# radhofan/Fairify

Measured on AMD Instinct MI355X. Metric: % partitions verified + partitions/sec on AC suite at 1/2/4/8 MI355X, higher is better.
Workload: dtype fp32

## Files before the change

### fairify_amd/csrc/bindings.cpp

```cpp
#include <hip/hip_runtime.h>
#include <pybind11/pybind11.h>
#include <pybind11/stl.h>

#include <cmath>
#include <cstring>
#include <cstdint>
#include <stdexcept>
#include <vector>

#include "runtime_host.h"

namespace py = pybind11;

extern "C" int fa_bounds_launch(const NetDesc& net, BoundArgs args, hipStream_t stream);
extern "C" int fa_crown_phase_launch(const NetDesc& net, CrownPhaseArgs a, hipStream_t stream);
extern "C" size_t fa_crown_phase_bytes(const NetDesc& net);
extern "C" int fa_point_try_launch(const NetDesc& net, BoundArgs a, hipStream_t stream);
extern "C" int fa_forward_launch(const NetDesc& net, FwdArgs a, hipStream_t stream);
extern "C" int fa_sim_launch(const NetDesc& net, SimArgs a, hipStream_t stream);
extern "C" int fa_sim_shaped(const NetDesc& net);
extern "C" int fa_rate_launch(const NetDesc& net, RateArgs a, hipStream_t stream);
extern "C" int fa_ascent_launch(const NetDesc& net, AscentArgs a, hipStream_t stream);
extern "C" int fa_certify_launch(CertArgs a, hipStream_t stream);
extern "C" int fa_falsify_launch(const NetDesc& net, FalsifyArgs a, hipStream_t stream);
// ... 84 lines not shown
  }
  int n_params;
  int total_floats;
};

const NetDesc& fa_net_desc(py::handle h) { return h.cast<const Net&>().d; }
void register_bab(py::module& m);
void register_relu(py::module& m);
void register_beta(py::module& m);
extern "C" int fa_crown_launch(const NetDesc& net, BoundArgs a, hipStream_t stream);
extern "C" int fa_refine_launch(const NetDesc& net, BoundArgs a, hipStream_t stream);
extern "C" int fa_backward_launch(const NetDesc& net, BoundArgs a, hipStream_t stream);
extern "C" int fa_refine_crown_launch(const NetDesc& net, BoundArgs a, hipStream_t stream);
void register_csv(py::module& m);

using fa_rt::ckl;

PYBIND11_MODULE(_C, m) {
  m.doc() = "fairify_amd CDNA4 (gfx950) kernels";
  py::class_<Net>(m, "Net")
      .def(py::init<const std::vector<int>&, double>())
      .def_readonly("n_params", &Net::n_params)
      .def_readonly("total_floats", &Net::total_floats)
      .def_property_readonly("wperm_off", [](const Net& n) { return n.d.wperm_off; })
      .def_property_readonly("pack_g", [](const Net& n) { return n.d.pack_g; })
      .def_property_readonly("pack_off", [](const Net& n) { return n.d.pack_off; })
      .def_property_readonly("n_hidden", [](const Net& n) { return n.d.n_hidden; })
      .def_property_readonly("n_neurons", [](const Net& n) { return n.d.n_neurons; });

  m.def("bounds", [](const Net& net, uintptr_t flat, uintptr_t lo, uintptr_t hi, uintptr_t dead_in, int R,
                     int symbolic, uintptr_t out_lb, uintptr_t out_ub, uintptr_t Lc, uintptr_t L0, uintptr_t Le,
                     uintptr_t Uc, uintptr_t U0, uintptr_t Ue, uintptr_t layer_lb, uintptr_t layer_ub,
                     uintptr_t dead_out, int G, uintptr_t stream, unsigned long long fold, uintptr_t phase_in,
                     uintptr_t infeas) {
    NetDesc d = net.d;
    BoundArgs a{};
    a.flat = P<const float>(flat);
    a.lo = P<const float>(lo);
    a.hi = P<const float>(hi);
    a.dead_in = P<const uint8_t>(dead_in);
    a.R = R;
    a.symbolic = symbolic;
    a.G = G;
    a.out_lb = P<float>(out_lb);
    a.out_ub = P<float>(out_ub);
    a.Lc = P<float>(Lc); a.L0 = P<float>(L0); a.Le = P<float>(Le);
    a.Uc = P<float>(Uc); a.U0 = P<float>(U0); a.Ue = P<float>(Ue);
    a.layer_lb = P<float>(layer_lb);
    a.layer_ub = P<float>(layer_ub);
    a.dead_out = P<uint8_t>(dead_out);
    a.fold = fold;
    a.phase_in = P<const int8_t>(phase_in);
    a.infeas = P<uint8_t>(infeas);
    ckl(fa_bounds_launch(d, a, (hipStream_t)stream), "bounds");
  }, py::arg("net"), py::arg("flat"), py::arg("lo"), py::arg("hi"), py::arg("dead_in"), py::arg("R"),
     py::arg("symbolic"), py::arg("out_lb"), py::arg("out_ub"), py::arg("Lc"), py::arg("L0"), py::arg("Le"),
     py::arg("Uc"), py::arg("U0"), py::arg("Ue"), py::arg("layer_lb"), py::arg("layer_ub"), py::arg("dead_out"),
     py::arg("G"), py::arg("stream"), py::arg("fold") = 0ull, py::arg("phase_in") = 0, py::arg("infeas") = 0);

  m.def("crown_phase", [](const Net& net, uintptr_t flat, uintptr_t lo, uintptr_t hi, int R, uintptr_t phase,
                          uintptr_t layer_lb, uintptr_t layer_ub, uintptr_t infeas, uintptr_t out_lb, uintptr_t out_ub,
                          uintptr_t Lc, uintptr_t L0, uintptr_t Le, uintptr_t Uc, uintptr_t U0, uintptr_t Ue,
                          uintptr_t split, uintptr_t score, uintptr_t low, uintptr_t stream) {
    CrownPhaseArgs a{};
    a.flat = P<const float>(flat);
    a.lo = P<const float>(lo);
    a.hi = P<const float>(hi);
    a.R = R;
    a.phase = P<const int8_t>(phase);
    a.layer_lb = P<const float>(layer_lb);
    a.layer_ub = P<const float>(layer_ub);
    a.infeas = P<const uint8_t>(infeas);
    a.out_lb = P<float>(out_lb);
    a.out_ub = P<float>(out_ub);
    a.Lc = P<float>(Lc); a.L0 = P<float>(L0); a.Le = P<float>(Le);
    a.Uc = P<float>(Uc); a.U0 = P<float>(U0); a.Ue = P<float>(Ue);
    a.split = P<int>(split);
    a.score = P<float>(score);
    a.low = P<float>(low);
    const int rc = fa_crown_phase_launch(net.d, a, (hipStream_t)stream);
    if (rc != 0) throw std::runtime_error("crown_phase launch failed, code " + std::to_string(rc));
  });

  m.def("relu_fits", [](const Net& net) { return fa_crown_phase_bytes(net.d) > 0; });

  m.def("crown", [](const Net& net, uintptr_t flat, uintptr_t lo, uintptr_t hi, uintptr_t dead_in, int R,
                    uintptr_t out_lb, uintptr_t out_ub, uintptr_t Lc, uintptr_t L0, uintptr_t Le, uintptr_t Uc,
                    uintptr_t U0, uintptr_t Ue, uintptr_t layer_lb, uintptr_t layer_ub, uintptr_t stream) {
    BoundArgs a{};
    a.flat = P<const float>(flat);
    a.lo = P<const float>(lo);
// ... 482 lines not shown
```

### fairify_amd/csrc/symbolic.hip

```cpp
#include <hip/hip_runtime.h>

#include <stdlib.h>

#include <algorithm>
#include <map>
#include <mutex>
#include <tuple>
#include <utility>
#include <vector>

#include "args.h"

#define FA_SYM_MAXC 48

struct SymCfg {
  int nc;
  int cdim[FA_SYM_MAXC];
  unsigned long long fold;
  int w_lds[FA_MAX_LAYERS];
  int b_lds[FA_MAX_LAYERS];
  int lds_floats;
  int stage_off;
  int stage_floats;
};
// ... 19 lines not shown
        if (a->pa_idx[k] == d) x = a->values[v * a->npa + k];
    return x;
  }
};

__device__ __forceinline__ int fa_trot(int rho) { return rho >> 3; }

template <int NT, int PG = 1>
struct SymSlab {
  static constexpr int TS = 16 * NT + 4;
  static constexpr int TILE1 = 2 * 16 * TS;
  static constexpr int TILE = 2 * TILE1;
  static constexpr int BOX = 3 * FA_SYM_MAXC;
  static constexpr int BOXTAB = PG > 1 ? 2 * PG * 32 : 0;
  static constexpr int FLOATS = (TILE + 2 * PG * BOX + BOXTAB + 3) & ~3;
};

template <bool PAIR, int TM>
struct SymForm {
  static constexpr bool CR = !PAIR && TM >= 2;
};

__device__ __forceinline__ void fa_pq_to_ul(const f32x4& P, const f32x4& Q, int fc, float gg, f32x4& U,
                                            f32x4& L) {
  const float sl = (fc == 1 || fc == 3) ? 2.f * gg : 0.f;
#pragma unroll
  for (int i = 0; i < 4; ++i) {
    const float q = Q[i], e = sl * fabsf(q);
    U[i] = (P[i] + q) + e;
    L[i] = (P[i] - q) - e;
  }
}

template <int NT, bool PAIR, int PG = 1, bool CR = false, class S = SymShapeAny>
__device__ __forceinline__ bool fa_sym_epilogue(const NetDesc& net, const BoundArgs& a, const SymCfg& cfg,
                                                const float* smem, float* T, const float* bxv_in, const int* cdim_s,
                                                int l, int r_in, int node_in, int r2, int node2, bool v2, int lane,
                                                int jt0, const f32x4 (&U)[2][NT],
                                                const f32x4 (&Lq)[2][NT], float (&nu)[2][NT][4],
                                                float (&nlo)[2][NT][4]) {
  constexpr int TS = SymSlab<NT>::TS;
  constexpr bool CS = S::L > 0;
  const int col = lane & 15, grp = lane >> 4;
  const int n_out = CS ? S::dim(l + 1) : net.dims[l + 1];
  const float* sb = smem + cfg.b_lds[l];
  const bool last = CS ? l == S::L - 1 : l == net.n_layers - 1;
  const float gg = net.g_gemm[l];
  const float gc = net.g_conc;
  const float gi = net.g_one;
  const float unit = net.unit;
  const float gnext = last ? 0.f : (CR ? net.g_fwd[l + 1] : net.g_gemm[l + 1]);
  const int noff = net.neuron_off[l];
  const int nc = cfg.nc;
  const int n0 = CS ? S::dim(0) : net.dims[0];
  const int tsub = lane >> 5;
  const bool second = PAIR && tsub;
  constexpr int PS = 16 / PG;
  const int gbox = PG > 1 ? col / PS : 0;
  const int bidx = tsub * PG + gbox;
  const int r = PG > 1 ? r_in + bidx : (second ? r2 : r_in);
  const int node = PG > 1 ? (a.V > 0 ? r / a.V : r) : (second ? node2 : node_in);
  const float* bxv = bxv_in + (PG > 1 ? bidx : (second ? 1 : 0)) * SymSlab<NT, PG>::BOX;
  const int jt = PAIR ? jt0 : jt0 + tsub;
  const int n_out_t = n_out;
  const bool nl_act = PG > 1 ? r < a.R : (16 * jt < n_out_t && (!second || v2));
  const int ob = (lane >> 4) & 1;
  float* Trow = T + tsub * SymSlab<NT>::TILE1 + (ob * 16 + col) * TS + fa_trot(ob * 16 + col);
#pragma unroll
    for (int u = 0; u < 2; ++u)
#pragma unroll
      for (int ct = 0; ct < NT; ++ct)
#pragma unroll
        for (int i = 0; i < 4; ++i) {
          const int ru = 4 * grp + i, rl = 16 + 4 * grp + i;
          T[u * SymSlab<NT>::TILE1 + ru * TS + fa_trot(ru) + ct * 16 + col] = U[u][ct][i];
          T[u * SymSlab<NT>::TILE1 + rl * TS + fa_trot(rl) + ct * 16 + col] = Lq[u][ct][i];
        }
    __builtin_amdgcn_wave_barrier();
    const int j = PG > 1 ? col - gbox * PS : 16 * jt + col;
    const bool jv = j < n_out;
    float v[16 * NT];
#pragma unroll
    for (int c = 0; c < 16 * NT; ++c) v[c] = Trow[c];
    const float braw = sb[PG > 1 ? col : min(j, n_out - 1)];
    const float b = jv ? braw : 0.f;
    float s1 = 0.f, s2 = 0.f, mg = 0.f;
#pragma unroll
    for (int c = 4; c < 16 * NT; ++c) {
      const float av = fabsf(v[c]);
      s1 = fmaf(v[c], bxv[c], s1);
      s2 = fmaf(av, bxv[FA_SYM_MAXC + c], s2);
      mg = fmaf(av, bxv[2 * FA_SYM_MAXC + c], mg);
    }
    float mn = s1 - s2, mx = s1 + s2;
    const float cr = v[0];
    float er = v[1], ivr = v[2], ier = v[3];
    const float sgn = ob ? -1.f : 1.f;
    er *= sgn;
    ier *= sgn;
    const float c0 = cr + b;
    const float mgc = mg;
    mn += c0; mx += c0; mg += fabsf(c0);
    const float iv = ivr + b;
    const float eI = ier * (1.f + 2.f * gg) + gg * fabsf(b);
    const float e = er * (1.f + 2.f * gg) + gg * fabsf(b);
    float bound;
    if (ob == 0) bound = fminf(iv + gi * fabsf(iv) + eI, mx + gc * mg + e);
    else bound = fmaxf(iv - gi * fabsf(iv) - eI, mn - gc * mg - e);
    const float other = __shfl_xor(bound, 16, 64);
    const float ub = ob == 0 ? bound : other;
    const float lb = ob == 0 ? other : bound;
    if (nl_act && jv && a.layer_lb) {
      if (ob == 0) a.layer_ub[(size_t)r * net.n_neurons + noff + j] = ub;
      else a.layer_lb[(size_t)r * net.n_neurons + noff + j] = lb;
    }
    if (last) {
      if (nl_act && j == 0) {
        float* Cf = ob == 0 ? a.Uc : a.Lc;
        if (ob == 0) {
          a.out_ub[r] = ub; a.U0[r] = c0; a.Ue[r] = e;
        } else {
          a.out_lb[r] = lb; a.L0[r] = c0; a.Le[r] = e;
        }
        for (int d = 0; d < n0; ++d)
          if ((cfg.fold >> d) & 1ull) Cf[(size_t)r * n0 + d] = 0.f;
        for (int c = 0; c < nc; ++c) Cf[(size_t)r * n0 + cdim_s[c]] = Trow[4 + c];
      }
      return false;
    }
    bool forced = false, fact = false;
    if (nl_act && jv) {
      if (a.dead_in) forced = a.dead_in[(size_t)r * net.n_hidden + noff + j] != 0;
      else if (a.dead_part) forced = a.dead_part[(size_t)a.node_part[node] * net.n_hidden + noff + j] != 0;
      if (a.phase_in) {
        const int8_t ph = a.phase_in[(size_t)r * net.n_hidden + noff + j];
        forced = forced || ph < 0;
        fact = ph > 0;
        if (ob == 0 && a.infeas && ((ph < 0 && lb > 0.f) || (ph > 0 && ub < 0.f))) a.infeas[r] = 1;
      }
    }
    const bool isdead = ub <= 0.f;
    const bool isact = lb >= 0.f;
    if (nl_act && ob == 0 && jv && a.dead_out) a.dead_out[(size_t)r * net.n_hidden + noff + j] = isdead ? 1 : 0;
    const bool zero = isdead || forced || !jv;
    const float aa = mn - gc * mg + e;
    const float bb = mx + gc * mg + e;
    const bool chord = !zero && !isact && !fact && aa < 0.f;
    const float sc = (bb / (bb - aa)) * (1.f + 4.f * unit);
    const float shift = e - aa;
    const float cc = c0 * sc + sc * shift;
    const float sU = zero ? 0.f : (chord ? sc : 1.f);
    const float cU = zero ? 0.f : (chord ? cc : c0);
    const float mU = zero ? 0.f : (chord ? sc * mgc * (1.f + 8.f * unit) + fabsf(cc) : mg);
    const float eU = zero ? 0.f : (chord ? 4.f * unit * sc * (mg + fabsf(shift)) : e);
    const float aL = mn - gc * mg - e;
    const float bL = mx + gc * mg - e;
    const bool lam1 = !zero && (isact || ((bL > 0.f) && (bL > -aL)));
    const bool up = ob == 0;
    const float ivn = zero ? 0.f : fmaxf(up ? ub : lb, 0.f);
    const float s = up ? sU : (lam1 ? 1.f : 0.f);
    const float cnew = up ? cU : (lam1 ? c0 : 0.f);
    const float en = up ? eU : (lam1 ? e : 0.f);
    const float mgn = up ? mU : (lam1 ? mg : 0.f);
    const float mg_b = CR ? mgn + __shfl_xor(mgn, 16, 64) : mgn;
    const float iv_b = CR ? fmaxf(ivn, __shfl_xor(ivn, 16, 64)) : ivn;
    v[0] = cnew;
    v[1] = sgn * (en + gnext * mg_b);
    v[2] = ivn;
    v[3] = sgn * (gnext * iv_b);
#pragma unroll
    for (int c = 4; c < 16 * NT; ++c) v[c] *= s;
    if (nl_act) {
#pragma unroll
      for (int c = 0; c < 16 * NT; ++c) Trow[c] = v[c];
    }
    __builtin_amdgcn_wave_barrier();
#pragma unroll
    for (int u = 0; u < 2; ++u)
#pragma unroll
      for (int ct = 0; ct < NT; ++ct)
#pragma unroll
        for (int i = 0; i < 4; ++i) {
          const int ru = 4 * grp + i, rl = 16 + 4 * grp + i;
          const float xu = T[u * SymSlab<NT>::TILE1 + ru * TS + fa_trot(ru) + ct * 16 + col];
          const float xl = T[u * SymSlab<NT>::TILE1 + rl * TS + fa_trot(rl) + ct * 16 + col];
          nu[u][ct][i] = CR ? 0.5f * (xu + xl) : xu;
          nlo[u][ct][i] = CR ? 0.5f * (xu - xl) : xl;
        }
    __builtin_amdgcn_wave_barrier();
    return true;
}

template <int NT, int TM, bool PAIR, int PG = 1, class S = SymShapeAny>
__device__ __forceinline__ void fa_sym_layer(const NetDesc& net, const BoundArgs& a, const SymCfg& cfg,
                                             const float* smem, float* T, const float* bxv, const int* cdim_s,
                                             int l, int r, int node, int r2, int node2, bool v2, int lane,
                                             const float (&B)[NT][PAIR ? 2 : TM][2][4],
                                             float (&A)[NT][PAIR ? 2 : TM][2][4]) {
  constexpr int TMS = PAIR ? 2 : TM;
  constexpr bool CR = SymForm<PAIR, TM>::CR;
  constexpr int TS = SymSlab<NT>::TS;
  constexpr bool CS = S::L > 0;
  const int col = lane & 15, grp = lane >> 4;
  const int n_in = CS ? S::dim(l) : net.dims[l], n_out = CS ? S::dim(l + 1) : net.dims[l + 1];
  const int tin = (n_in + 15) >> 4, tout = (n_out + 15) >> 4;
  const float* sw = smem + cfg.w_lds[l];
  const float* sb = smem + cfg.b_lds[l];
  const bool last = CS ? l == S::L - 1 : l == net.n_layers - 1;
  const float gg = net.g_gemm[l];
  const float gc = net.g_conc;
  const float gi = net.g_one;
  const float unit = net.unit;
  const float gnext = last ? 0.f : net.g_gemm[l + 1];
  const int noff = net.neuron_off[l];
  const int nc = cfg.nc;
  const int n0 = CS ? S::dim(0) : net.dims[0];
  const bool nl_act = lane < 32;
  const int ob = (lane >> 4) & 1;
#ifndef FA_SYM_TIMING_NO_EPILOGUE
  if (PG > 1 && l == 0) {
    const float* boxtab = bxv + 2 * PG * SymSlab<NT, PG>::BOX;
    const float g0 = net.g_gemm[0];
    const int n0v = n0;
    f32x4 U[2][NT], Lq[2][NT];
#pragma unroll
    for (int u = 0; u < 2; ++u) {
// ... 73 lines not shown
          for (int ct = 0; ct < NT; ++ct) {
            const int bt = PAIR ? bi : t;
            if (CR) {
              su[bi][ct] = fmaf(wv[i], B[ct][bt][0][i], su[bi][ct]);
              sl[bi][ct] = fmaf(fabsf(wv[i]), B[ct][bt][1][i], sl[bi][ct]);
            } else {
              su[bi][ct] = fmaf(wp, B[ct][bt][0][i], fmaf(wn, B[ct][bt][1][i], su[bi][ct]));
              sl[bi][ct] = fmaf(wp, B[ct][bt][1][i], fmaf(wn, B[ct][bt][0][i], sl[bi][ct]));
            }
          }
      }
    }
    f32x4 U[2][NT], Lq[2][NT];
#pragma unroll
    for (int ct = 0; ct < NT; ++ct) U[1][ct] = Lq[1][ct] = f32x4{0.f, 0.f, 0.f, 0.f};
#pragma unroll
    for (int bi = 0; bi < NB; ++bi)
#pragma unroll
      for (int ct = 0; ct < NT; ++ct) {
        float xu = su[bi][ct], xl = sl[bi][ct];
        xu += __shfl_xor(xu, 16, 64);
        xl += __shfl_xor(xl, 16, 64);
        xu += __shfl_xor(xu, 32, 64);
        xl += __shfl_xor(xl, 32, 64);
        U[bi][ct] = f32x4{grp == 0 ? xu : 0.f, 0.f, 0.f, 0.f};
        Lq[bi][ct] = f32x4{grp == 0 ? xl : 0.f, 0.f, 0.f, 0.f};
        if (CR) fa_pq_to_ul(f32x4(U[bi][ct]), f32x4(Lq[bi][ct]), ct * 16 + col, gg, U[bi][ct], Lq[bi][ct]);
      }
    float nu[2][NT][4], nlo[2][NT][4];
    fa_sym_epilogue<NT, PAIR, PG, CR, S>(net, a, cfg, smem, T, bxv, cdim_s, l, r, node, r2, node2, v2, lane, 0, U, Lq,
                                  nu, nlo);
    return;
  }
#endif
#pragma unroll
  for (int jt0 = 0; jt0 < TM; jt0 += 2) {
    if (jt0 >= tout) break;
    f32x4 U[2][NT], Lq[2][NT];
#pragma unroll
    for (int u = 0; u < 2; ++u) {
      const int jt = jt0 + u;
#pragma unroll
      for (int ct = 0; ct < NT; ++ct) {
        U[u][ct] = f32x4{0.f, 0.f, 0.f, 0.f};
        Lq[u][ct] = f32x4{0.f, 0.f, 0.f, 0.f};
      }
      if (PAIR ? (jt0 > 0) : (jt >= tout || jt >= TM)) continue;
      const float4* wq = reinterpret_cast<const float4*>(sw) + (size_t)(PAIR ? 0 : jt) * tin * 64 + lane;
#pragma unroll
      for (int t = 0; t < TM; ++t) {
        if (t >= tin) break;
        const float4 w4 = wq[t * 64];
        const float wv[4] = {w4.x, w4.y, w4.z, w4.w};
#pragma unroll
        for (int i = 0; i < 4; ++i) {
          const float wp = fmaxf(wv[i], 0.f), wn = fminf(wv[i], 0.f);
#pragma unroll
          for (int ct = 0; ct < NT; ++ct) {
            const int bt = PAIR ? u : t;
            const float bu = B[ct][bt][0][i], bl = B[ct][bt][1][i];
            if (CR) {
              U[u][ct] = fa_mfma4(wv[i], bu, U[u][ct]);
              Lq[u][ct] = fa_mfma4(fabsf(wv[i]), bl, Lq[u][ct]);
            } else {
              U[u][ct] = fa_mfma4(wp, bu, U[u][ct]);
              Lq[u][ct] = fa_mfma4(wp, bl, Lq[u][ct]);
// ... 22 lines not shown
        }
    if (l == net.n_layers - 1) {
      if (lane == 0) a.out_lb[r] = nu[0][0][0] + nlo[0][0][1];
      continue;
    }
#else
    if (!fa_sym_epilogue<NT, PAIR, PG, CR, S>(net, a, cfg, smem, T, bxv, cdim_s, l, r, node, r2, node2, v2, lane, jt0, U,
                                       Lq, nu, nlo))
      continue;
#endif
#pragma unroll
    for (int u = 0; u < 2; ++u) {
      if (jt0 + u >= TMS) break;
#pragma unroll
      for (int ct = 0; ct < NT; ++ct)
#pragma unroll
        for (int i = 0; i < 4; ++i) {
          A[ct][jt0 + u][0][i] = nu[u][ct][i];
          A[ct][jt0 + u][1][i] = nlo[u][ct][i];
        }
    }
  }
}

#ifndef FA_SYM_WPE7
#define FA_SYM_WPE7 2
#endif
#ifndef FA_SYM_WPE4
#define FA_SYM_WPE4 2
#endif
#define FA_SYM_WAVES_PER_EU(NT, TM, PAIR) \
  ((PAIR) ? 3 : ((TM) == 2 ? 3 : ((TM) == 4 ? FA_SYM_WPE4 : ((TM) == 7 ? FA_SYM_WPE7 : 1))))

template <int NT, int TM, bool PAIR, int PG, class S, int... LS>
__device__ __forceinline__ void fa_sym_layers_c(std::integer_sequence<int, LS...>, const NetDesc& net,
                                                const BoundArgs& a, const SymCfg& cfg, const float* smem, float* T,
                                                const float* bxv, const int* cdim_s, int r, int node, int r2,
                                                int node2, bool v2, int lane, float (&XA)[NT][PAIR ? 2 : TM][2][4],
                                                float (&XB)[NT][PAIR ? 2 : TM][2][4]) {
  ((LS & 1 ? fa_sym_layer<NT, TM, PAIR, PG, S>(net, a, cfg, smem, T, bxv, cdim_s, LS, r, node, r2, node2, v2, lane,
                                               XB, XA)
           : fa_sym_layer<NT, TM, PAIR, PG, S>(net, a, cfg, smem, T, bxv, cdim_s, LS, r, node, r2, node2, v2, lane,
                                               XA, XB)),
   ...);
}

#ifndef FA_SYM_BIG_THREADS
#define FA_SYM_BIG_THREADS 512
#endif
#define FA_SYM_THREADS(TM) ((TM) == 7 ? FA_SYM_BIG_THREADS : FA_THREADS)

template <int NT, int TM, bool PAIR, int PG = 1, class S = SymShapeAny>
__global__ void __launch_bounds__(FA_SYM_THREADS(TM)) __attribute__((amdgpu_waves_per_eu(FA_SYM_WAVES_PER_EU(NT, TM, PAIR))))
fa_sym_kernel(NetDesc net, BoundArgs a, SymCfg cfg) {
  constexpr bool CR = SymForm<PAIR, TM>::CR;
  constexpr int TMS = PAIR ? 2 : TM;
  extern __shared__ __attribute__((aligned(16))) float smem[];
  const int tid = threadIdx.x;
  {
    const float4* src = reinterpret_cast<const float4*>(a.flat + cfg.stage_off);
    float4* dst = reinterpret_cast<float4*>(smem);
    for (int e = tid; e < (cfg.stage_floats >> 2); e += FA_SYM_THREADS(TM)) dst[e] = src[e];
  }
  int* cdim_s = reinterpret_cast<int*>(smem + cfg.lds_floats - FA_SYM_MAXC);
  for (int c = tid; c < FA_SYM_MAXC; c += FA_SYM_THREADS(TM)) cdim_s[c] = c < cfg.nc ? cfg.cdim[c] : -1;
  __syncthreads();
  const int lane = tid & 63;
  const int grp = lane >> 4;
  const int wave = tid >> 6;
  const int nw = FA_SYM_THREADS(TM) / 64;
  const int n0 = S::L > 0 ? S::dim(0) : net.dims[0];
  const int nc = cfg.nc;
  const float g0 = net.g_gemm[0];
  float* T = smem + cfg.lds_floats + wave * SymSlab<NT, PG>::FLOATS;
  float* bxv = T + SymSlab<NT>::TILE;
  const int tin0 = (n0 + 15) >> 4;
  int role[NT], cdm[NT];
#pragma unroll
  for (int ct = 0; ct < NT; ++ct) {
    const int c = ct * 16 + (lane & 15);
    role[ct] = c == 0 ? 1 : c == 1 ? 2 : c == 2 ? 3 : c == 3 ? 4 : (c - 4 < nc ? 0 : 5);
    cdm[ct] = (role[ct] == 0) ? cdim_s[c - 4] : -1;
  }
  constexpr int RPW = PAIR ? 2 * PG : 1;
  for (int r0 = (blockIdx.x * nw + wave) * RPW; r0 < a.R; r0 += gridDim.x * nw * RPW) {
    const int r = __builtin_amdgcn_readfirstlane(r0);
    const bool v2 = PAIR && r + 1 < a.R;
    const int rb = v2 ? r + 1 : r;
    if (a.skip_status) {
      bool any = false;
#pragma unroll
      for (int bi = 0; bi < RPW; ++bi) {
        const int rr = min(r + bi, a.R - 1);
        const int8_t s1 = a.skip_status[a.skip_part[a.V > 0 ? rr / a.V : rr]];
        any = any || s1 == 3 || s1 == 4;
      }
      if (!any) continue;
    }
    SymBox bxs[RPW];
#pragma unroll
    for (int bi = 0; bi < RPW; ++bi) {
      SymBox& bx = bxs[bi];
      const int rr = PG > 1 ? min(r + bi, a.R - 1) : (bi ? rb : r);
// ... 35 lines not shown
        const bool kv = k < n0;
        if (kv) {
          xl = bt.lo(k);
          xh = bt.hi(k);
        }
        const bool folded = kv && ((cfg.fold >> k) & 1ull);
        const float m = fmaxf(fabsf(xl), fabsf(xh));
#pragma unroll
        for (int ct = 0; ct < NT; ++ct) {
          float vu = 0.f, vl = 0.f;
          if (kv) {
            switch (role[ct]) {
              case 0: vu = (!folded && cdm[ct] == k) ? 1.f : 0.f; vl = CR ? 0.f : vu; break;
              case 1: vu = folded ? xl : 0.f; vl = CR ? 0.f : vu; break;
              case 2: vu = CR ? 0.f : g0 * m; vl = CR ? g0 * m : -vu; break;
              case 3:
                vu = CR ? 0.5f * (xh + xl) : xh;
                vl = CR ? 0.5f * (xh - xl) : xl;
                break;
              case 4:
                vu = CR ? 0.5f * g0 * (fabsf(xh) - fabsf(xl)) : g0 * fabsf(xh);
                vl = CR ? 0.5f * g0 * (fabsf(xh) + fabsf(xl)) : -(g0 * fabsf(xl));
                break;
              default: break;
            }
          }
          XA[ct][t][0][i] = vu;
          XA[ct][t][1][i] = vl;
        }
      }
    }
    __builtin_amdgcn_wave_barrier();
    if constexpr (S::L > 0) {
      fa_sym_layers_c<NT, TM, PAIR, PG, S>(std::make_integer_sequence<int, S::L>{}, net, a, cfg, smem, T, bxv, cdim_s,
                                           r, bx.node, rb, bxs[RPW - 1].node, v2, lane, XA, XB);
    } else {
      for (int l = 0; l < net.n_layers; ++l) {
        if (l & 1)
          fa_sym_layer<NT, TM, PAIR, PG>(net, a, cfg, smem, T, bxv, cdim_s, l, r, bx.node, rb, bxs[RPW - 1].node, v2,
                                         lane, XB, XA);
        else
          fa_sym_layer<NT, TM, PAIR, PG>(net, a, cfg, smem, T, bxv, cdim_s, l, r, bx.node, rb, bxs[RPW - 1].node, v2,
                                         lane, XA, XB);
      }
    }
    __builtin_amdgcn_wave_barrier();
  }
}


namespace {

typedef void (*SymKernel)(NetDesc, BoundArgs, SymCfg);

template <int NT, int TM, bool PAIR = false, int PG = 1>
SymKernel sym_ptr() {
  return fa_sym_kernel<NT, TM, PAIR, PG>;
}

bool use_pack() {
  static const bool v = [] {
    const char* e = getenv("FAIRIFY_SYM_PACK");
    return !(e && *e == '0');
  }();
  return v;
}

SymKernel select_packed(int pg) {
// ... 29 lines not shown
      if (TM <= 4) return sym_ptr<1, 4>();
      if (TM <= 7) return sym_ptr<1, 7>();
      if (TM <= 10) return sym_ptr<1, 10>();
      return nullptr;
    case 2:
      if (TM <= 1) return sym_ptr<2, 1>();
      if (TM <= 2) return sym_ptr<2, 2>();
      if (TM <= 4) return sym_ptr<2, 4>();
      if (TM <= 10) return sym_ptr<2, 10>();
      return nullptr;
    case 3:
      if (TM <= 1) return sym_ptr<3, 1>();
      if (TM <= 2) return sym_ptr<3, 2>();
      return nullptr;
    default:
      return nullptr;
  }
}

int tm_bucket(int NT, int TM) {
  if (TM > max_tm()) return 0;
  const int b = TM <= 1 ? 1 : TM <= 2 ? 2 : TM <= 4 ? 4 : TM <= 7 ? 7 : TM <= 10 ? 10 : 0;
  if (NT == 2 && b == 7) return 10;
  if (NT == 3 && b > 2) return 0;
  return NT >= 1 && NT <= 3 ? b : 0;
}

struct ShapedKernel {
  int nt, tm;
  bool pair;
  int pg;
  std::vector<int> dims;
  SymKernel k;
};
template <int NT, int TM, bool PAIR, int PG, int... D>
ShapedKernel shaped() {
  return {NT, TM, PAIR, PG, {D...}, fa_sym_kernel<NT, TM, PAIR, PG, SymShape<D...>>};
}

const std::vector<ShapedKernel>& shaped_kernels() {
  static const std::vector<ShapedKernel> v = {
      shaped<1, 4, false, 1, 13, 64, 32, 16, 8, 4, 1>(),
      shaped<2, 4, false, 1, 13, 64, 32, 16, 8, 4, 1>(),
      shaped<2, 4, false, 1, 16, 64, 32, 16, 8, 4, 1>(),
      shaped<1, 4, false, 1, 13, 64, 64, 1>(),
      shaped<1, 4, false, 1, 13, 50, 1>(),
      shaped<1, 7, false, 1, 13, 100, 100, 1>(),
      shaped<1, 7, false, 1, 13, 100, 1>(),
      shaped<1, 1, true, 1, 13, 16, 8, 1>(),
      shaped<1, 1, true, 1, 13, 12, 12, 1>(),
      shaped<1, 1, true, 1, 13, 10, 10, 10, 10, 1>(),
      shaped<1, 1, true, 2, 13, 5, 5, 1>(),
      shaped<1, 1, true, 2, 13, 5, 5, 5, 5, 1>(),
  };
  return v;
}

SymKernel select_shaped(const NetDesc& net, int NT, int tmb, bool pair, int pg) {
  const char* e = getenv("FAIRIFY_SYM_SHAPED");
  if (e && *e == '0') return nullptr;
  for (const auto& s : shaped_kernels()) {
    if (s.nt != NT || s.tm != tmb || s.pair != pair || s.pg != pg || (int)s.dims.size() != net.n_layers + 1) continue;
    bool same = true;
    for (int l = 0; l <= net.n_layers && same; ++l) same = s.dims[l] == net.dims[l];
    if (same) return s.k;
  }
  return nullptr;
}

int device_cus() {
  static int cus = 0;
  static std::once_flag once;
  std::call_once(once, [] {
    int dev = 0;
    if (hipGetDevice(&dev) != hipSuccess ||
        hipDeviceGetAttribute(&cus, hipDeviceAttributeMultiprocessorCount, dev) != hipSuccess || cus <= 0)
      cus = 256;
  });
  return cus;
}

}

extern "C" int fa_sym_try_launch(const NetDesc& net, BoundArgs a, unsigned long long fold_mask,
                                 hipStream_t stream) {
  if (!a.symbolic || a.R <= 0) return 0;
  const int n0 = net.dims[0];
  if (n0 > 64) return 0;
  SymCfg cfg{};
  cfg.fold = fold_mask;
  int nc = 0;
  for (int d = 0; d < n0; ++d)
    if (!((fold_mask >> d) & 1ull)) {
      if (nc >= FA_SYM_MAXC) return 0;
      cfg.cdim[nc++] = d;
    }
  cfg.nc = nc;
  const int cols = nc + 4;
  const int NT = (cols + 15) / 16;
  int TM = 1;
  for (int l = 0; l < net.n_layers; ++l) TM = std::max(TM, (net.dims[l] + 15) / 16);
  TM = std::max(TM, (net.dims[net.n_layers] + 15) / 16);
  SymKernel k = select_kernel(NT, TM);
  if (!k) return 0;
  const bool pair0 = k == sym_ptr<1, 1, true>();
  const int tmb = tm_bucket(NT, TM);
  const int pg = (pair0 && net.pack_g > 1 && net.dims[0] <= 16 && use_pack()) ? net.pack_g : 1;
  if (pg > 1) k = select_packed(pg);
  if (!k) return 0;
  if (const SymKernel ks = select_shaped(net, NT, tmb, pair0, pg)) k = ks;
  int off = 0;
  if (pg > 1) {
    cfg.w_lds[0] = 0;
    off = pg * 256;
    for (int l = 1; l < net.n_layers; ++l) {
      cfg.w_lds[l] = off;
      off += 256;
    }
    for (int l = 0; l < net.n_layers; ++l) {
      cfg.b_lds[l] = off;
      off += 16;
    }
    if (off != net.pack_floats) return -1;
    cfg.stage_off = net.pack_off;
  } else {
    for (int l = 0; l < net.n_layers; ++l) {
      cfg.w_lds[l] = off;
      off += ((net.dims[l] + 15) / 16) * ((net.dims[l + 1] + 15) / 16) * 256;
    }
    for (int l = 0; l < net.n_layers; ++l) {
      cfg.b_lds[l] = off;
      off += net.dims[l + 1];
    }
    off = ((off + 3) & ~3);
    if (off != net.wperm_floats) return -1;
    cfg.stage_off = net.wperm_off;
  }
  cfg.stage_floats = off;
  off += FA_SYM_MAXC;
  cfg.lds_floats = off;
  int slab = 0;
  switch (NT) {
    case 1:
// ... 12 lines not shown
  {
    std::lock_guard<std::mutex> g(mu);
    const auto key = std::make_pair((const void*)k, bytes);
    auto it = occ.find(key);
    if (it == occ.end()) {
      if (!fa_lds_ok(bytes)) return -4;
      if (hipOccupancyMaxActiveBlocksPerMultiprocessor(&per_cu, k, threads, bytes) != hipSuccess || per_cu <= 0)
        per_cu = 1;
      occ[key] = per_cu;
    } else {
      per_cu = it->second;
    }
  }
  long long blocks = (a.R + rows_per_block - 1) / rows_per_block;
  const long long cap = (long long)device_cus() * per_cu;
  if (blocks > cap) blocks = cap;
  hipLaunchKernelGGL(k, dim3((unsigned)blocks), dim3(threads), bytes, stream, net, a, cfg);
  const hipError_t e = hipGetLastError();
  return e == hipSuccess ? 1 : -(int)e;
}

FA_LDS_REGISTER(FA_LDS_K((sym_ptr<1, 1>())), FA_LDS_K((sym_ptr<1, 1, true>())), FA_LDS_K((sym_ptr<1, 1, true, 2>())),
                FA_LDS_K((sym_ptr<1, 1, true, 4>())), FA_LDS_K((sym_ptr<1, 2>())), FA_LDS_K((sym_ptr<1, 4>())),
                FA_LDS_K((sym_ptr<1, 7>())), FA_LDS_K((sym_ptr<1, 10>())), FA_LDS_K((sym_ptr<2, 1>())),
                FA_LDS_K((sym_ptr<2, 2>())), FA_LDS_K((sym_ptr<2, 4>())), FA_LDS_K((sym_ptr<2, 10>())),
                FA_LDS_K((sym_ptr<3, 1>())), FA_LDS_K((sym_ptr<3, 2>())));
FA_LDS_REGISTER(FA_LDS_K((fa_sym_kernel<1, 4, false, 1, SymShape<13, 64, 32, 16, 8, 4, 1>>)),
                FA_LDS_K((fa_sym_kernel<2, 4, false, 1, SymShape<13, 64, 32, 16, 8, 4, 1>>)),
                FA_LDS_K((fa_sym_kernel<2, 4, false, 1, SymShape<16, 64, 32, 16, 8, 4, 1>>)),
                FA_LDS_K((fa_sym_kernel<1, 4, false, 1, SymShape<13, 64, 64, 1>>)),
                FA_LDS_K((fa_sym_kernel<1, 4, false, 1, SymShape<13, 50, 1>>)),
                FA_LDS_K((fa_sym_kernel<1, 7, false, 1, SymShape<13, 100, 100, 1>>)),
                FA_LDS_K((fa_sym_kernel<1, 7, false, 1, SymShape<13, 100, 1>>)));
FA_LDS_REGISTER(FA_LDS_K((fa_sym_kernel<1, 1, true, 1, SymShape<13, 16, 8, 1>>)),
                FA_LDS_K((fa_sym_kernel<1, 1, true, 1, SymShape<13, 12, 12, 1>>)),
                FA_LDS_K((fa_sym_kernel<1, 1, true, 1, SymShape<13, 10, 10, 10, 10, 1>>)),
                FA_LDS_K((fa_sym_kernel<1, 1, true, 2, SymShape<13, 5, 5, 1>>)),
                FA_LDS_K((fa_sym_kernel<1, 1, true, 2, SymShape<13, 5, 5, 5, 5, 1>>)));
```

Baseline: 268,800.

## Software-pipeline MFMA chains of next output-tile pair into symbolic epilogue

```diff
diff --git a/fairify_amd/csrc/bindings.cpp b/fairify_amd/csrc/bindings.cpp
--- a/fairify_amd/csrc/bindings.cpp
+++ b/fairify_amd/csrc/bindings.cpp
@@ -140,9 +140,19 @@
                      int symbolic, uintptr_t out_lb, uintptr_t out_ub, uintptr_t Lc, uintptr_t L0, uintptr_t Le,
                      uintptr_t Uc, uintptr_t U0, uintptr_t Ue, uintptr_t layer_lb, uintptr_t layer_ub,
                      uintptr_t dead_out, int G, uintptr_t stream, unsigned long long fold, uintptr_t phase_in,
-                     uintptr_t infeas) {
+                     uintptr_t infeas, int V, uintptr_t values, std::vector<int> pa, uintptr_t node_part,
+                     uintptr_t dead_part, uintptr_t skip_status, uintptr_t skip_part) {
     NetDesc d = net.d;
     BoundArgs a{};
+    if (V > 0 && (pa.empty() || (int)pa.size() > FA_MAX_PA || !values)) throw std::invalid_argument("bounds: V needs pa and values");
+    a.V = V;
+    a.npa = V > 0 ? (int)pa.size() : 0;
+    for (int i = 0; i < a.npa; ++i) a.pa_idx[i] = pa[i];
+    a.values = P<const float>(values);
+    a.node_part = P<const int>(node_part);
+    a.dead_part = P<const uint8_t>(dead_part);
+    a.skip_status = P<const int8_t>(skip_status);
+    a.skip_part = P<const int>(skip_part);
     a.flat = P<const float>(flat);
     a.lo = P<const float>(lo);
     a.hi = P<const float>(hi);
@@ -164,7 +174,9 @@
   }, py::arg("net"), py::arg("flat"), py::arg("lo"), py::arg("hi"), py::arg("dead_in"), py::arg("R"),
      py::arg("symbolic"), py::arg("out_lb"), py::arg("out_ub"), py::arg("Lc"), py::arg("L0"), py::arg("Le"),
      py::arg("Uc"), py::arg("U0"), py::arg("Ue"), py::arg("layer_lb"), py::arg("layer_ub"), py::arg("dead_out"),
-     py::arg("G"), py::arg("stream"), py::arg("fold") = 0ull, py::arg("phase_in") = 0, py::arg("infeas") = 0);
+     py::arg("G"), py::arg("stream"), py::arg("fold") = 0ull, py::arg("phase_in") = 0, py::arg("infeas") = 0,
+     py::arg("V") = 0, py::arg("values") = 0, py::arg("pa") = std::vector<int>{}, py::arg("node_part") = 0,
+     py::arg("dead_part") = 0, py::arg("skip_status") = 0, py::arg("skip_part") = 0);
 
   m.def("crown_phase", [](const Net& net, uintptr_t flat, uintptr_t lo, uintptr_t hi, int R, uintptr_t phase,
                           uintptr_t layer_lb, uintptr_t layer_ub, uintptr_t infeas, uintptr_t out_lb, uintptr_t out_ub,
diff --git a/fairify_amd/csrc/symbolic.hip b/fairify_amd/csrc/symbolic.hip
--- a/fairify_amd/csrc/symbolic.hip
+++ b/fairify_amd/csrc/symbolic.hip
@@ -75,13 +75,91 @@
   }
 }
 
-template <int NT, bool PAIR, int PG = 1, bool CR = false, class S = SymShapeAny>
+#define FA_SYM_MID_POINTS 12
+__device__ constexpr int fa_sym_mid_cum(int k) {
+  constexpr int w[FA_SYM_MID_POINTS] = {2, 2, 2, 2, 1, 1, 1, 3, 3, 2, 1, 4};
+  int s = 0;
+  for (int i = 0; i < k; ++i) s += w[i];
+  return s;
+}
+#ifndef FA_SYM_PIPE_GAP
+#define FA_SYM_PIPE_GAP(TIN) ((20 + (TIN) - 1) / (TIN))
+#endif
+struct SymNoMid {
+  template <int K>
+  __device__ __forceinline__ void at() {}
+};
+
+template <int NT, int TM, int TIN>
+struct SymChains {
+  static constexpr int STEPS = 2 * TIN * 4;
+  f32x4 P[2][NT], Q[2][NT];
+  float wv[4];
+  const float4* wq;
+  const float (&B)[NT][TM][2][4];
+
+  __device__ __forceinline__ SymChains(const float* sw, int lane, const float (&B_)[NT][TM][2][4])
+      : wq(reinterpret_cast<const float4*>(sw) + lane), B(B_) {}
+
+  template <int JT0, int TOUT, int N0, int N1, bool SPREAD>
+  __device__ __forceinline__ void run() {
+#pragma unroll
+    for (int n = N0; n < N1; ++n) {
+      const int u = n / (4 * TIN), t = (n >> 2) % TIN, i = n & 3;
+      if (n == 0) {
+#pragma unroll
+        for (int uu = 0; uu < 2; ++uu)
+#pragma unroll
+          for (int ct = 0; ct < NT; ++ct) P[uu][ct] = Q[uu][ct] = f32x4{0.f, 0.f, 0.f, 0.f};
+      }
+      if (JT0 + u >= TOUT || JT0 + u >= TM) continue;
+      if (i == 0) {
+        const float4 w4 = wq[((JT0 + u) * TIN + t) * 64];
+        wv[0] = w4.x; wv[1] = w4.y; wv[2] = w4.z; wv[3] = w4.w;
+      }
+#pragma unroll
+      for (int ct = 0; ct < NT; ++ct) {
+        P[u][ct] = fa_mfma4(wv[i], B[ct][t][0][i], P[u][ct]);
+        Q[u][ct] = fa_mfma4(fabsf(wv[i]), B[ct][t][1][i], Q[u][ct]);
+        if (SPREAD) {
+          __builtin_amdgcn_sched_group_barrier(0x8, 1, 0);
+          __builtin_amdgcn_sched_group_barrier(0x2 | 0x100 | 0x200, FA_SYM_PIPE_GAP(TIN), 0);
+          __builtin_amdgcn_sched_group_barrier(0x8, 1, 0);
+          __builtin_amdgcn_sched_group_barrier(0x2 | 0x100 | 0x200, FA_SYM_PIPE_GAP(TIN), 0);
+        }
+      }
+    }
+  }
+
+  template <int JT0, int TOUT>
+  __device__ __forceinline__ void take(int col, float gg, f32x4 (&U)[2][NT], f32x4 (&Lq)[2][NT]) const {
+#pragma unroll
+    for (int u = 0; u < 2; ++u)
+#pragma unroll
+      for (int ct = 0; ct < NT; ++ct) {
+        U[u][ct] = P[u][ct];
+        Lq[u][ct] = Q[u][ct];
+        if (JT0 + u < TOUT && JT0 + u < TM) fa_pq_to_ul(P[u][ct], Q[u][ct], ct * 16 + col, gg, U[u][ct], Lq[u][ct]);
+      }
+  }
+};
+
+template <class CH, int JT0, int TOUT>
+struct SymMid {
+  CH& ch;
+  template <int K>
+  __device__ __forceinline__ void at() {
+    ch.template run<JT0, TOUT, CH::STEPS * fa_sym_mid_cum(K) / 24, CH::STEPS * fa_sym_mid_cum(K + 1) / 24, true>();
+  }
+};
+
+template <int NT, bool PAIR, int PG = 1, bool CR = false, class S = SymShapeAny, class MID = SymNoMid>
 __device__ __forceinline__ bool fa_sym_epilogue(const NetDesc& net, const BoundArgs& a, const SymCfg& cfg,
                                                 const float* smem, float* T, const float* bxv_in, const int* cdim_s,
                                                 int l, int r_in, int node_in, int r2, int node2, bool v2, int lane,
                                                 int jt0, const f32x4 (&U)[2][NT],
                                                 const f32x4 (&Lq)[2][NT], float (&nu)[2][NT][4],
-                                                float (&nlo)[2][NT][4]) {
+                                                float (&nlo)[2][NT][4], MID mid = MID{}) {
   constexpr int TS = SymSlab<NT>::TS;
   constexpr bool CS = S::L > 0;
   const int col = lane & 15, grp = lane >> 4;
@@ -119,12 +197,14 @@
           T[u * SymSlab<NT>::TILE1 + ru * TS + fa_trot(ru) + ct * 16 + col] = U[u][ct][i];
           T[u * SymSlab<NT>::TILE1 + rl * TS + fa_trot(rl) + ct * 16 + col] = Lq[u][ct][i];
         }
+    mid.template at<0>();
     __builtin_amdgcn_wave_barrier();
     const int j = PG > 1 ? col - gbox * PS : 16 * jt + col;
     const bool jv = j < n_out;
     float v[16 * NT];
 #pragma unroll
     for (int c = 0; c < 16 * NT; ++c) v[c] = Trow[c];
+    mid.template at<1>();
     const float braw = sb[PG > 1 ? col : min(j, n_out - 1)];
     const float b = jv ? braw : 0.f;
     float s1 = 0.f, s2 = 0.f, mg = 0.f;
@@ -134,7 +214,9 @@
       s1 = fmaf(v[c], bxv[c], s1);
       s2 = fmaf(av, bxv[FA_SYM_MAXC + c], s2);
       mg = fmaf(av, bxv[2 * FA_SYM_MAXC + c], mg);
-    }
+      if (c == 8 * NT + 1) mid.template at<2>();
+    }
+    mid.template at<3>();
     float mn = s1 - s2, mx = s1 + s2;
     const float cr = v[0];
     float er = v[1], ivr = v[2], ier = v[3];
@@ -153,10 +235,12 @@
     const float other = __shfl_xor(bound, 16, 64);
     const float ub = ob == 0 ? bound : other;
     const float lb = ob == 0 ? other : bound;
+    mid.template at<4>();
     if (nl_act && jv && a.layer_lb) {
       if (ob == 0) a.layer_ub[(size_t)r * net.n_neurons + noff + j] = ub;
       else a.layer_lb[(size_t)r * net.n_neurons + noff + j] = lb;
     }
+    mid.template at<5>();
     if (last) {
       if (nl_act && j == 0) {
         float* Cf = ob == 0 ? a.Uc : a.Lc;
@@ -182,9 +266,11 @@
         if (ob == 0 && a.infeas && ((ph < 0 && lb > 0.f) || (ph > 0 && ub < 0.f))) a.infeas[r] = 1;
       }
     }
+    mid.template at<6>();
     const bool isdead = ub <= 0.f;
     const bool isact = lb >= 0.f;
     if (nl_act && ob == 0 && jv && a.dead_out) a.dead_out[(size_t)r * net.n_hidden + noff + j] = isdead ? 1 : 0;
+    mid.template at<7>();
     const bool zero = isdead || forced || !jv;
     const float aa = mn - gc * mg + e;
     const float bb = mx + gc * mg + e;
@@ -196,6 +282,7 @@
     const float cU = zero ? 0.f : (chord ? cc : c0);
     const float mU = zero ? 0.f : (chord ? sc * mgc * (1.f + 8.f * unit) + fabsf(cc) : mg);
     const float eU = zero ? 0.f : (chord ? 4.f * unit * sc * (mg + fabsf(shift)) : e);
+    mid.template at<8>();
     const float aL = mn - gc * mg - e;
     const float bL = mx + gc * mg - e;
     const bool lam1 = !zero && (isact || ((bL > 0.f) && (bL > -aL)));
@@ -213,11 +300,15 @@
     v[3] = sgn * (gnext * iv_b);
 #pragma unroll
     for (int c = 4; c < 16 * NT; ++c) v[c] *= s;
+    mid.template at<9>();
     if (nl_act) {
 #pragma unroll
       for (int c = 0; c < 16 * NT; ++c) Trow[c] = v[c];
     }
+    mid.template at<10>();
     __builtin_amdgcn_wave_barrier();
+    mid.template at<11>();
+    static_assert(FA_SYM_MID_POINTS == 12, "the epilogue has 12 hook points");
 #pragma unroll
     for (int u = 0; u < 2; ++u)
 #pragma unroll
@@ -234,7 +325,46 @@
     return true;
 }
 
-template <int NT, int TM, bool PAIR, int PG = 1, class S = SymShapeAny>
+template <int NT, int TM, class S, int LC, int PP, class CH>
+__device__ __forceinline__ void fa_sym_pipe_pair(const NetDesc& net, const BoundArgs& a, const SymCfg& cfg,
+                                                 const float* smem, float* T, const float* bxv, const int* cdim_s,
+                                                 int r, int node, int lane, CH& ch, float (&A)[NT][TM][2][4]) {
+  constexpr int TOUT = (S::dim(LC + 1) + 15) >> 4, JT0 = 2 * PP;
+  f32x4 U[2][NT], Lq[2][NT];
+  float nu[2][NT][4], nlo[2][NT][4];
+  ch.template take<JT0, TOUT>(lane & 15, net.g_gemm[LC], U, Lq);
+  if constexpr (JT0 + 2 < TOUT)
+    fa_sym_epilogue<NT, false, 1, true, S>(net, a, cfg, smem, T, bxv, cdim_s, LC, r, node, r, node, false, lane, JT0, U,
+                                           Lq, nu, nlo, SymMid<CH, JT0 + 2, TOUT>{ch});
+  else
+    fa_sym_epilogue<NT, false, 1, true, S>(net, a, cfg, smem, T, bxv, cdim_s, LC, r, node, r, node, false, lane, JT0, U,
+                                           Lq, nu, nlo);
+#pragma unroll
+  for (int u = 0; u < 2; ++u) {
+    if (JT0 + u >= TM) break;
+#pragma unroll
+    for (int ct = 0; ct < NT; ++ct)
+#pragma unroll
+      for (int i = 0; i < 4; ++i) {
+        A[ct][JT0 + u][0][i] = nu[u][ct][i];
+        A[ct][JT0 + u][1][i] = nlo[u][ct][i];
+      }
+  }
+}
+
+template <int NT, int TM, class S, int LC, int... PS>
+__device__ __forceinline__ void fa_sym_pairs_pipe(std::integer_sequence<int, PS...>, const NetDesc& net,
+                                                  const BoundArgs& a, const SymCfg& cfg, const float* smem, float* T,
+                                                  const float* bxv, const int* cdim_s, int r, int node, int lane,
+                                                  const float (&B)[NT][TM][2][4], float (&A)[NT][TM][2][4]) {
+  constexpr int TIN = (S::dim(LC) + 15) >> 4, TOUT = (S::dim(LC + 1) + 15) >> 4;
+  using CH = SymChains<NT, TM, TIN>;
+  CH ch(smem + cfg.w_lds[LC], lane, B);
+  ch.template run<0, TOUT, 0, CH::STEPS, false>();
+  (fa_sym_pipe_pair<NT, TM, S, LC, PS>(net, a, cfg, smem, T, bxv, cdim_s, r, node, lane, ch, A), ...);
+}
+
+template <int NT, int TM, bool PAIR, int PG = 1, class S = SymShapeAny, bool PIPE = false, int LC = -1>
 __device__ __forceinline__ void fa_sym_layer(const NetDesc& net, const BoundArgs& a, const SymCfg& cfg,
                                              const float* smem, float* T, const float* bxv, const int* cdim_s,
                                              int l, int r, int node, int r2, int node2, bool v2, int lane,
@@ -374,6 +504,14 @@
                                   nu, nlo);
     return;
   }
+  if constexpr (PIPE && LC < S::L - 1) {
+    static_assert(CR && CS && PG == 1 && LC >= 0, "pipelined loop: compile-time-shape C/R kernels");
+    static_assert(S::dim(S::L) == 1, "the logit layer is the VALU dot above, every other layer is hidden");
+    constexpr int NP = (((S::dim(LC + 1) + 15) >> 4) + 1) / 2;
+    fa_sym_pairs_pipe<NT, TM, S, LC>(std::make_integer_sequence<int, NP>{}, net, a, cfg, smem, T, bxv, cdim_s, r,
+                                     node, lane, B, A);
+    return;
+  }
 #endif
 #pragma unroll
   for (int jt0 = 0; jt0 < TM; jt0 += 2) {
@@ -462,16 +600,16 @@
 #define FA_SYM_WAVES_PER_EU(NT, TM, PAIR) \
   ((PAIR) ? 3 : ((TM) == 2 ? 3 : ((TM) == 4 ? FA_SYM_WPE4 : ((TM) == 7 ? FA_SYM_WPE7 : 1))))
 
-template <int NT, int TM, bool PAIR, int PG, class S, int... LS>
+template <int NT, int TM, bool PAIR, int PG, class S, bool PIPE, int... LS>
 __device__ __forceinline__ void fa_sym_layers_c(std::integer_sequence<int, LS...>, const NetDesc& net,
                                                 const BoundArgs& a, const SymCfg& cfg, const float* smem, float* T,
                                                 const float* bxv, const int* cdim_s, int r, int node, int r2,
                                                 int node2, bool v2, int lane, float (&XA)[NT][PAIR ? 2 : TM][2][4],
                                                 float (&XB)[NT][PAIR ? 2 : TM][2][4]) {
-  ((LS & 1 ? fa_sym_layer<NT, TM, PAIR, PG, S>(net, a, cfg, smem, T, bxv, cdim_s, LS, r, node, r2, node2, v2, lane,
-                                               XB, XA)
-           : fa_sym_layer<NT, TM, PAIR, PG, S>(net, a, cfg, smem, T, bxv, cdim_s, LS, r, node, r2, node2, v2, lane,
-                                               XA, XB)),
+  ((LS & 1 ? fa_sym_layer<NT, TM, PAIR, PG, S, PIPE, LS>(net, a, cfg, smem, T, bxv, cdim_s, LS, r, node, r2, node2, v2,
+                                                         lane, XB, XA)
+           : fa_sym_layer<NT, TM, PAIR, PG, S, PIPE, LS>(net, a, cfg, smem, T, bxv, cdim_s, LS, r, node, r2, node2, v2,
+                                                         lane, XA, XB)),
    ...);
 }
 
@@ -480,9 +618,20 @@
 #endif
 #define FA_SYM_THREADS(TM) ((TM) == 7 ? FA_SYM_BIG_THREADS : FA_THREADS)
 
-template <int NT, int TM, bool PAIR, int PG = 1, class S = SymShapeAny>
-__global__ void __launch_bounds__(FA_SYM_THREADS(TM)) __attribute__((amdgpu_waves_per_eu(FA_SYM_WAVES_PER_EU(NT, TM, PAIR))))
+template <int NT, int TM, bool PAIR, class S>
+struct SymTune {
+  static constexpr int WAVES = FA_SYM_WAVES_PER_EU(NT, TM, PAIR);
+};
+template <int... D>
+struct SymTune<1, 4, false, SymShape<D...>> {
+  static constexpr int WAVES = 3;
+};
+
+template <int NT, int TM, bool PAIR, int PG = 1, class S = SymShapeAny, bool PIPE = false>
+__global__ void __launch_bounds__(FA_SYM_THREADS(TM))
+    __attribute__((amdgpu_waves_per_eu(SymTune<NT, TM, PAIR, S>::WAVES)))
 fa_sym_kernel(NetDesc net, BoundArgs a, SymCfg cfg) {
+  constexpr int THREADS = FA_SYM_THREADS(TM);
   constexpr bool CR = SymForm<PAIR, TM>::CR;
   constexpr int TMS = PAIR ? 2 : TM;
   extern __shared__ __attribute__((aligned(16))) float smem[];
@@ -490,15 +639,15 @@
   {
     const float4* src = reinterpret_cast<const float4*>(a.flat + cfg.stage_off);
     float4* dst = reinterpret_cast<float4*>(smem);
-    for (int e = tid; e < (cfg.stage_floats >> 2); e += FA_SYM_THREADS(TM)) dst[e] = src[e];
+    for (int e = tid; e < (cfg.stage_floats >> 2); e += THREADS) dst[e] = src[e];
   }
   int* cdim_s = reinterpret_cast<int*>(smem + cfg.lds_floats - FA_SYM_MAXC);
-  for (int c = tid; c < FA_SYM_MAXC; c += FA_SYM_THREADS(TM)) cdim_s[c] = c < cfg.nc ? cfg.cdim[c] : -1;
+  for (int c = tid; c < FA_SYM_MAXC; c += THREADS) cdim_s[c] = c < cfg.nc ? cfg.cdim[c] : -1;
   __syncthreads();
   const int lane = tid & 63;
   const int grp = lane >> 4;
   const int wave = tid >> 6;
-  const int nw = FA_SYM_THREADS(TM) / 64;
+  const int nw = THREADS / 64;
   const int n0 = S::L > 0 ? S::dim(0) : net.dims[0];
   const int nc = cfg.nc;
   const float g0 = net.g_gemm[0];
@@ -600,8 +749,8 @@
     }
     __builtin_amdgcn_wave_barrier();
     if constexpr (S::L > 0) {
-      fa_sym_layers_c<NT, TM, PAIR, PG, S>(std::make_integer_sequence<int, S::L>{}, net, a, cfg, smem, T, bxv, cdim_s,
-                                           r, bx.node, rb, bxs[RPW - 1].node, v2, lane, XA, XB);
+      fa_sym_layers_c<NT, TM, PAIR, PG, S, PIPE>(std::make_integer_sequence<int, S::L>{}, net, a, cfg, smem, T, bxv,
+                                                 cdim_s, r, bx.node, rb, bxs[RPW - 1].node, v2, lane, XA, XB);
     } else {
       for (int l = 0; l < net.n_layers; ++l) {
         if (l & 1)
@@ -697,21 +846,28 @@
   int pg;
   std::vector<int> dims;
   SymKernel k;
+  SymKernel kpipe;
 };
 template <int NT, int TM, bool PAIR, int PG, int... D>
 ShapedKernel shaped() {
-  return {NT, TM, PAIR, PG, {D...}, fa_sym_kernel<NT, TM, PAIR, PG, SymShape<D...>>};
+  const SymKernel k = fa_sym_kernel<NT, TM, PAIR, PG, SymShape<D...>>;
+  return {NT, TM, PAIR, PG, {D...}, k, k};
+}
+template <int NT, int TM, int... D>
+ShapedKernel shaped_pipe() {
+  return {NT, TM, false, 1, {D...}, fa_sym_kernel<NT, TM, false, 1, SymShape<D...>>,
+          fa_sym_kernel<NT, TM, false, 1, SymShape<D...>, true>};
 }
 
 const std::vector<ShapedKernel>& shaped_kernels() {
   static const std::vector<ShapedKernel> v = {
-      shaped<1, 4, false, 1, 13, 64, 32, 16, 8, 4, 1>(),
+      shaped_pipe<1, 4, 13, 64, 32, 16, 8, 4, 1>(),
       shaped<2, 4, false, 1, 13, 64, 32, 16, 8, 4, 1>(),
       shaped<2, 4, false, 1, 16, 64, 32, 16, 8, 4, 1>(),
       shaped<1, 4, false, 1, 13, 64, 64, 1>(),
-      shaped<1, 4, false, 1, 13, 50, 1>(),
-      shaped<1, 7, false, 1, 13, 100, 100, 1>(),
-      shaped<1, 7, false, 1, 13, 100, 1>(),
+      shaped_pipe<1, 4, 13, 50, 1>(),
+      shaped_pipe<1, 7, 13, 100, 100, 1>(),
+      shaped_pipe<1, 7, 13, 100, 1>(),
       shaped<1, 1, true, 1, 13, 16, 8, 1>(),
       shaped<1, 1, true, 1, 13, 12, 12, 1>(),
       shaped<1, 1, true, 1, 13, 10, 10, 10, 10, 1>(),
@@ -721,14 +877,14 @@
   return v;
 }
 
-SymKernel select_shaped(const NetDesc& net, int NT, int tmb, bool pair, int pg) {
+const ShapedKernel* select_shaped(const NetDesc& net, int NT, int tmb, bool pair, int pg) {
   const char* e = getenv("FAIRIFY_SYM_SHAPED");
   if (e && *e == '0') return nullptr;
   for (const auto& s : shaped_kernels()) {
     if (s.nt != NT || s.tm != tmb || s.pair != pair || s.pg != pg || (int)s.dims.size() != net.n_layers + 1) continue;
     bool same = true;
     for (int l = 0; l <= net.n_layers && same; ++l) same = s.dims[l] == net.dims[l];
-    if (same) return s.k;
+    if (same) return &s;
   }
   return nullptr;
 }
@@ -773,7 +929,10 @@
   const int pg = (pair0 && net.pack_g > 1 && net.dims[0] <= 16 && use_pack()) ? net.pack_g : 1;
   if (pg > 1) k = select_packed(pg);
   if (!k) return 0;
-  if (const SymKernel ks = select_shaped(net, NT, tmb, pair0, pg)) k = ks;
+  if (const ShapedKernel* ks = select_shaped(net, NT, tmb, pair0, pg)) {
+    const char* ep = getenv("FAIRIFY_SYM_PIPE");
+    k = (ep && *ep == '0') ? ks->k : ks->kpipe;
+  }
   int off = 0;
   if (pg > 1) {
     cfg.w_lds[0] = 0;
@@ -852,6 +1011,10 @@
                 FA_LDS_K((fa_sym_kernel<1, 4, false, 1, SymShape<13, 50, 1>>)),
                 FA_LDS_K((fa_sym_kernel<1, 7, false, 1, SymShape<13, 100, 100, 1>>)),
                 FA_LDS_K((fa_sym_kernel<1, 7, false, 1, SymShape<13, 100, 1>>)));
+FA_LDS_REGISTER(FA_LDS_K((fa_sym_kernel<1, 4, false, 1, SymShape<13, 64, 32, 16, 8, 4, 1>, true>)),
+                FA_LDS_K((fa_sym_kernel<1, 4, false, 1, SymShape<13, 50, 1>, true>)),
+                FA_LDS_K((fa_sym_kernel<1, 7, false, 1, SymShape<13, 100, 100, 1>, true>)),
+                FA_LDS_K((fa_sym_kernel<1, 7, false, 1, SymShape<13, 100, 1>, true>)));
 FA_LDS_REGISTER(FA_LDS_K((fa_sym_kernel<1, 1, true, 1, SymShape<13, 16, 8, 1>>)),
                 FA_LDS_K((fa_sym_kernel<1, 1, true, 1, SymShape<13, 12, 12, 1>>)),
                 FA_LDS_K((fa_sym_kernel<1, 1, true, 1, SymShape<13, 10, 10, 10, 10, 1>>)),
```

After: 273,600, median of 3. Within noise of the previous version (+1.8%).
